# zhangkao/IIP_UAVSal_Saliency

Hardware: AMD Instinct MI355X
Metric: saliency frames/sec at 360x640 (higher is better)
Workload: dtype f32; 1 GPU; 360x640 batch=1 clip(s)/GPU seq=8, UAVSal.forward_clips, prec=f32, launch loop; requests_in_flight=1, clips_per_gpu=1, seq_len=8, height=360, width=640, precision=f32, persistent_state=False, parallelism=single GPU, fused_dw=10

## Files before the change

iip_uavsal_saliency_amd/_lib.py:

```python
from __future__ import annotations

import collections
import ctypes as C
import os

PKG = os.path.dirname(os.path.abspath(__file__))
LIB_PATH = os.environ.get("UAVSAL_HIP_LIB") or os.path.join(PKG, "libuavsal_hip.so")

PREC = {"f32": 0, "bf16x3": 1, "bf16": 2, "f16x3": 3}
ACT_NONE, ACT_RELU6, ACT_SIGMOID = 0, 1, 2
EPI_AFFINE, EPI_TWA, EPI_LSTM = 0, 1, 2
SK_TICKET_BASE = 4096

_ERR = {-1: "UAVSAL_EINVAL (null pointer / non-positive size)",
        -2: "UAVSAL_EALIGN (channel count / ld / pointer not 16-byte aligned)",
        -3: "UAVSAL_ESHAPE (shape not supported by the kernel)",
        -4: "UAVSAL_ESTATE (plan used in the wrong state)",
        -5: "UAVSAL_EDEVICE (a kernel reported a device-side error; the run's outputs are invalid)"}
ERR_STREAMK = 1
DW_KERNEL = {1: "dw3x3_kernel<1, 4, 4>", 2: "dw3x3_kernel<1, 2, 2>", 3: "dw3x3_kernel<2, 2, 2>", 4: "dw3x3_dilated_kernel",
             16: "dw3x3_map_lds_kernel<16, 256>", 32: "dw3x3_map_lds_kernel<32, 256>",
             528: "dw3x3_map_lds_kernel<16, 512>", 544: "dw3x3_map_lds_kernel<32, 512>",
             2048: "dw3x3_rowclass_kernel<256>"}

# ... 191 lines not shown
    _fields_ = [("g", _f), ("ldg", C.c_int32), ("carry", _f), ("z", _f), ("x", _f), ("ldx", C.c_int32),
                ("hprev", _f), ("ldh", C.c_int32), ("dz", _f), ("carry_out", _f), ("dx", _f),
                ("n_pix", C.c_int64), ("C", C.c_int32)]


class TwaWgradDesc(C.Structure):
    _fields_ = [("dz", _f), ("x", _f), ("ldx", C.c_int32), ("h", _f), ("ldh", C.c_int32), ("h0", _f), ("ldh0", C.c_int32),
                ("ws", _f), ("ws_bytes", C.c_int64), ("out", _f),
                ("T", C.c_int32), ("H", C.c_int32), ("W", C.c_int32), ("C", C.c_int32), ("accumulate", C.c_int32)]


class DecBwdDesc(C.Structure):
    _fields_ = [("gy", _f), ("gy_img_pitch", C.c_int64), ("gy_row_pitch", C.c_int64), ("gy_col_pitch", C.c_int64),
                ("y", _f), ("e", _f), ("d", _f), ("s1", _f), ("wd9", _f), ("s2", _f), ("w3", _f), ("s3", _f), ("ge", _f),
                ("n_img", C.c_int32), ("H", C.c_int32), ("W", C.c_int32), ("C", C.c_int32)]


TRAIN_DESC_TYPES = [TwaGateDesc, TwaWgradDesc, DecBwdDesc]

class PixGemmDesc(C.Structure):
    _fields_ = [("a", _f), ("lda", C.c_int32), ("b", _f), ("ldb", C.c_int32), ("row_scale", _f),
                ("w", _f), ("ldw", C.c_int32), ("rowdot", C.c_void_p), ("ws", _f), ("ws_bytes", C.c_int64),
                ("out", _f), ("ldo", C.c_int32), ("K", C.c_int64), ("M", C.c_int32), ("N", C.c_int32), ("accumulate", C.c_int32)]


class DecSumsDesc(C.Structure):
    _fields_ = [("gy", _f), ("gy_img_pitch", C.c_int64), ("gy_row_pitch", C.c_int64), ("gy_col_pitch", C.c_int64),
                ("y", _f), ("e", _f), ("d", _f), ("ga", _f), ("w3", _f), ("s3", _f),
                ("ws", C.c_void_p), ("ws_bytes", C.c_int64),
                ("n_img", C.c_int32), ("H", C.c_int32), ("W", C.c_int32), ("C", C.c_int32)]


class DecFinishDesc(C.Structure):
    _fields_ = [("ws", C.c_void_p), ("ws_bytes", C.c_int64), ("rowdot", C.c_void_p)] + [(n, _f) for n in (
        "wd", "w3", "s2", "s3", "r1", "mu1", "r2", "mu2", "r3", "mu3",
        "g_gamma1", "g_beta1", "g_wd", "g_gamma2", "g_beta2", "g_w3", "g_gamma3", "g_beta3")] + [
        ("C", C.c_int32), ("slabs", C.c_int32), ("accumulate", C.c_int32)]


DEC_NSUM = 12
TRAIN_DECODER_DESC_TYPES = [PixGemmDesc, DecSumsDesc, DecFinishDesc]

DESC_TYPES = [ConvDesc, DwDesc, StemDesc, BilinearDesc, TdiffDesc, TsumDesc, LayoutDesc, PostDesc, GuardDesc, CopyDesc,
              FusedIrDesc, WinoDesc, DwDotDesc, FillDesc, ScoreDesc, LetterboxDesc, OverlayDesc, GazeDesc, LossDesc, ConvRoute]

SYMBOLS = [
    ("uavsal_conv_gemm", C.c_int, [C.POINTER(ConvDesc), C.c_void_p]),
    ("uavsal_conv_route_of", C.c_int, [C.POINTER(ConvDesc), C.POINTER(ConvRoute)]),
    ("uavsal_conv_tile", C.c_int, [C.POINTER(ConvDesc)]),
    ("uavsal_conv_uses_split", C.c_int, [C.POINTER(ConvDesc)]),
    ("uavsal_conv_dwproj", C.c_int, [C.POINTER(ConvDesc)]),
    ("uavsal_streamk_workspace_bytes", C.c_longlong, []),
    ("uavsal_conv_streamk_grid", C.c_int, [C.POINTER(ConvDesc)]),
    ("uavsal_dw3x3", C.c_int, [C.POINTER(DwDesc), C.c_void_p]),
    ("uavsal_dw3x3_dot", C.c_int, [C.POINTER(DwDotDesc), C.c_void_p]),
    ("uavsal_dw_variant", C.c_int, [C.POINTER(DwDesc)]),
    ("uavsal_stem_conv", C.c_int, [C.POINTER(StemDesc), C.c_void_p]),
    ("uavsal_bilinear_ac", C.c_int, [C.POINTER(BilinearDesc), C.c_void_p]),
    ("uavsal_tdiff", C.c_int, [C.POINTER(TdiffDesc), C.c_void_p]),
    ("uavsal_tsum", C.c_int, [C.POINTER(TsumDesc), C.c_void_p]),
    ("uavsal_layout", C.c_int, [C.POINTER(LayoutDesc), C.c_void_p]),
    ("uavsal_postprocess", C.c_int, [C.POINTER(PostDesc), C.c_void_p]),
    ("uavsal_letterbox_u8", C.c_int, [C.POINTER(LetterboxDesc), C.c_void_p]),
    ("uavsal_overlay_workspace_bytes", C.c_int64, [C.POINTER(OverlayDesc)]),
    ("uavsal_overlay_u8", C.c_int, [C.POINTER(OverlayDesc), C.c_void_p]),
    ("uavsal_gaze_prepare", C.c_int, [C.POINTER(GazeDesc), C.c_void_p]),
    ("uavsal_loss_fu", C.c_int, [C.POINTER(LossDesc), C.c_void_p]),
    ("uavsal_loss_fu_grad", C.c_int, [C.POINTER(LossDesc), C.c_void_p]),
    ("uavsal_prior_accumulate", C.c_int, [C.POINTER(PriorAccDesc), C.c_void_p]),
    ("uavsal_prior_finish", C.c_int, [C.POINTER(PriorFinishDesc), C.c_void_p]),
    ("uavsal_prior_slab_frames", C.c_int, [C.c_int64, C.c_int32]),
    ("uavsal_prior_sizeof_desc", C.c_int, [C.c_int]),
    ("uavsal_twa_gate_bwd", C.c_int, [C.POINTER(TwaGateDesc), C.c_void_p]),
    ("uavsal_twa_wgrad_workspace_bytes", C.c_int64, [C.POINTER(TwaWgradDesc)]),
    ("uavsal_twa_wgrad_shares", C.c_int, [C.POINTER(TwaWgradDesc)]),
    ("uavsal_twa_wgrad", C.c_int, [C.POINTER(TwaWgradDesc), C.c_void_p]),
    ("uavsal_dec_bwd", C.c_int, [C.POINTER(DecBwdDesc), C.c_void_p]),
    ("uavsal_train_sizeof_desc", C.c_int, [C.c_int]),
    ("uavsal_pix_gemm_workspace_bytes", C.c_int64, [C.POINTER(PixGemmDesc)]),
    ("uavsal_pix_gemm_shares", C.c_int, [C.POINTER(PixGemmDesc)]),
    ("uavsal_pix_gemm", C.c_int, [C.POINTER(PixGemmDesc), C.c_void_p]),
    ("uavsal_dec_sums_workspace_bytes", C.c_int64, [C.POINTER(DecSumsDesc)]),
    ("uavsal_dec_sums_slabs", C.c_int, [C.POINTER(DecSumsDesc)]),
    ("uavsal_dec_sums_slab_rows", C.c_int, [C.POINTER(DecSumsDesc)]),
    ("uavsal_dec_sums", C.c_int, [C.POINTER(DecSumsDesc), C.c_void_p]),
    ("uavsal_dec_finish", C.c_int, [C.POINTER(DecFinishDesc), C.c_void_p]),
    ("uavsal_train_decoder_sizeof_desc", C.c_int, [C.c_int]),
    ("uavsal_guard", C.c_int, [C.POINTER(GuardDesc), C.c_void_p]),
    ("uavsal_copy_rows", C.c_int, [C.POINTER(CopyDesc), C.c_void_p]),
    ("uavsal_fill", C.c_int, [C.POINTER(FillDesc), C.c_void_p]),
    ("uavsal_plan_add_fill", C.c_int, [C.c_void_p, C.POINTER(FillDesc)]),
    ("uavsal_fused_ir", C.c_int, [C.POINTER(FusedIrDesc), C.c_void_p]),
    ("uavsal_fused_ir_supported", C.c_int, [C.POINTER(FusedIrDesc)]),
    ("uavsal_plan_add_fused_ir", C.c_int, [C.c_void_p, C.POINTER(FusedIrDesc)]),
    ("uavsal_wino_input", C.c_int, [C.POINTER(WinoDesc), C.c_void_p]),
    ("uavsal_wino_output", C.c_int, [C.POINTER(WinoDesc), C.c_void_p]),
    ("uavsal_plan_add_wino_input", C.c_int, [C.c_void_p, C.POINTER(WinoDesc)]),
    ("uavsal_plan_add_wino_output", C.c_int, [C.c_void_p, C.POINTER(WinoDesc)]),
    ("uavsal_plan_add_copy", C.c_int, [C.c_void_p, C.POINTER(CopyDesc)]),
    ("uavsal_plan_create", C.c_void_p, []),
    ("uavsal_plan_destroy", None, [C.c_void_p]),
    ("uavsal_plan_add_conv", C.c_int, [C.c_void_p, C.POINTER(ConvDesc)]),
    ("uavsal_plan_add_dw", C.c_int, [C.c_void_p, C.POINTER(DwDesc)]),
    ("uavsal_plan_add_dw_dot", C.c_int, [C.c_void_p, C.POINTER(DwDotDesc)]),
    ("uavsal_plan_add_stem", C.c_int, [C.c_void_p, C.POINTER(StemDesc)]),
    ("uavsal_plan_add_bilinear", C.c_int, [C.c_void_p, C.POINTER(BilinearDesc)]),
# ... 68 lines not shown
```

iip_uavsal_saliency_amd/build.py:

```python
from __future__ import annotations

import hashlib
import os
import subprocess
import sys
from concurrent.futures import ThreadPoolExecutor

PKG = os.path.dirname(os.path.abspath(__file__))
ROOT = os.path.dirname(PKG)
CSRC = os.path.join(PKG, "csrc")
INCLUDE = os.path.join(ROOT, "include")
LIB = os.path.join(PKG, "libuavsal_hip.so")
SOURCES = ["conv_gemm.hip", "conv_gemm_k32.hip", "dwproj.hip", "dw_conv.hip", "fused_ir.hip", "fused_mid.hip", "glue.hip", "letterbox.hip", "loss.hip", "overlay.hip", "post.hip", "plan.hip", "prior.hip", "score.hip", "train.hip", "train_decoder.hip", "winograd.hip"]
FLAGS = ["-O3", "--offload-arch=gfx950", "-std=c++17", "-fPIC", "-I" + INCLUDE, "-I" + CSRC]
FLAGS += os.environ.get("UAVSAL_EXTRA_HIPCC_FLAGS", "").split()


def _hipcc() -> str:
    for c in (os.environ.get("HIPCC"), "/opt/rocm/bin/hipcc", "hipcc"):
        if c and (os.path.isabs(c) and os.path.exists(c) or not os.path.isabs(c)):
            return c
    return "hipcc"


def _digest(paths, extra="") -> str:
    h = hashlib.sha256(extra.encode())
    for p in paths:
        h.update(os.path.basename(p).encode())
        with open(p, "rb") as f:
            h.update(f.read())
    return h.hexdigest()


def _stamp_ok(stamp: str, digest: str, target: str) -> bool:
    try:
        return os.path.exists(target) and open(stamp).read().strip() == digest
    except OSError:
        return False


def build(force: bool = False, verbose: bool = False) -> str:
    headers = sorted(os.path.join(CSRC, f) for f in os.listdir(CSRC) if f.endswith(".h"))
    headers += sorted(os.path.join(INCLUDE, f) for f in os.listdir(INCLUDE) if f.endswith(".h"))
    objs, jobs = [], []
    for src in SOURCES:
        s = os.path.join(CSRC, src)
        o = os.path.join(CSRC, src.replace(".hip", ".o"))
        objs.append(o)
        digest = _digest([s] + headers, " ".join(FLAGS))
        if force or not _stamp_ok(o + ".stamp", digest, o):
            jobs.append(([_hipcc()] + FLAGS + ["-c", s, "-o", o], o + ".stamp", digest))

    def run(job):
        cmd, stamp, digest = job
        if verbose:
            print(" ".join(cmd), flush=True)
        if stamp and os.path.exists(stamp):
            os.remove(stamp)
        r = subprocess.run(cmd, capture_output=True, text=True)
        if r.returncode != 0:
            raise RuntimeError("hipcc failed:\n%s\n%s" % (" ".join(cmd), r.stderr[-4000:]))
        if stamp:
            with open(stamp, "w") as f:
                f.write(digest)

    if jobs:
# ... 11 lines not shown
```

iip_uavsal_saliency_amd/csrc/conv_gemm.hip:

```cpp
#include <stdlib.h>
#include <type_traits>
#include "common.h"

#include "conv_gemm_common.h"
#include "conv_route.h"

namespace {

template <int PREC, int WAVES_M, int WAVES_N, int WM, int WN, int TAPS, bool FUSE = false>
__global__ __launch_bounds__(WAVES_M * WAVES_N * 64,
                             (WM * WN >= 4) ? ((PREC == UAVSAL_PREC_BF16X3 || PREC == UAVSAL_PREC_F16X3 || WAVES_M * WAVES_N == 8) ? 2 : 3) : 4)
void conv_gemm_kernel(const ConvK p) {
    constexpr int NT = WAVES_M * WAVES_N * 64;
    constexpr int NS = NT;
    static_assert(!FUSE || TAPS == 1, "the fused depthwise producer feeds a 1x1 projection");
    constexpr int BM = WAVES_M * WM * 32;
    constexpr int BN = WAVES_N * WN * 32;
    constexpr int KT = (PREC == UAVSAL_PREC_F32) ? 16 : 32;
    constexpr int NPAN = (PREC == UAVSAL_PREC_BF16X3 || PREC == UAVSAL_PREC_F16X3) ? 2 : 1;
    constexpr int NLD = (PREC == UAVSAL_PREC_F32) ? 1 : 2;
    constexpr int A_IT = (BM * 4) / NS;
    constexpr int B_IT = (BN * 4 + NS - 1) / NS;
    constexpr int APAN = BM * 64;
    constexpr int BPAN = BN * 64;
// ... 1087 lines not shown
    if (d->w_group_stride && !((tile == 8 || tile == 11) && k32_eligible(d, tile) && d->epi == UAVSAL_EPI_AFFINE && !d->a_split))
        status = UAVSAL_ESHAPE;
    else if (d->n_group < 0 || (d->n_group && !(k32_eligible(d, 11) && !d->a_split && !d->out_split)))
        status = UAVSAL_ESHAPE;
    const int ktiles = d->prec == UAVSAL_PREC_F32 ? (d->taps * d->Cin + 15) / 16 : (d->taps * d->Cin + 31) / 32;
    if (split_eligible(d, tile)) {
        r->family = UAVSAL_ROUTE_PRESPLIT;
        return status;
    }
    if (dwproj_eligible(d)) {
        r->family = UAVSAL_ROUTE_DWPROJ;
        r->dwproj = d->Cout > 128 ? 256 : (d->Cout > 64 ? 128 : (d->Cout > 32 ? 64 : 32));
        r->ksplit = dwproj_shares(d);
    } else if ((r->streamk = tile == 1 && sk1 >= 0 ? sk1 : streamk_plan(d, tile, ktiles)) > 0) {
        r->family = UAVSAL_ROUTE_STREAMK;
    } else if (tile >= 8 && tile <= 11) {
        r->family = UAVSAL_ROUTE_K32;
        r->ksplit = tile == 11 ? k32s_shares(d) : k32_shares(d, tile);
    } else if (d->prec == UAVSAL_PREC_F32 && !d->dw_w9c) {
        r->family = UAVSAL_ROUTE_F32_DMA;
    } else {
        r->family = UAVSAL_ROUTE_STAGED;
        r->ksplit = staged_shares(d, tile, ktiles);
    }
    if (r->ksplit > 1) r->reduce = r->family == UAVSAL_ROUTE_K32 && tile >= 10 ? UAVSAL_REDUCE_IN_LAUNCH : UAVSAL_REDUCE_LAUNCH;
    if (!status && r->family != UAVSAL_ROUTE_DWPROJ && !d->a) status = UAVSAL_EINVAL;
    return status;
}

extern "C" long long uavsal_streamk_workspace_bytes(void) {
    int dev = 0, n = 0;
    if (hipGetDevice(&dev) != hipSuccess ||
        hipDeviceGetAttribute(&n, hipDeviceAttributeMultiprocessorCount, dev) != hipSuccess || n <= 0) n = 256;
    const long long G = 2LL * n;
    return 65536 + G * 128 * 128 * 4;
}

extern "C" int uavsal_conv_route_of(const uavsal_conv_desc* d, uavsal_conv_route* r) {
    if (!d || !r || d->n_img <= 0 || d->H <= 0 || d->W <= 0 || d->Cout <= 0) return UAVSAL_EINVAL;
    (void)conv_route(d, r);
    return 0;
}

static uavsal_conv_route route_or_none(const uavsal_conv_desc* d, bool need_cin) {
    uavsal_conv_route r = {};
    if (d && (!need_cin || d->Cin > 0)) (void)uavsal_conv_route_of(d, &r);
    return r;
}
extern "C" int uavsal_conv_tile(const uavsal_conv_desc* d) { const int t = route_or_none(d, false).tile; return t ? t : UAVSAL_EINVAL; }
extern "C" int uavsal_conv_uses_split(const uavsal_conv_desc* d) { return route_or_none(d, true).family == UAVSAL_ROUTE_PRESPLIT; }
extern "C" int uavsal_conv_dwproj(const uavsal_conv_desc* d) { return route_or_none(d, true).dwproj; }
extern "C" int uavsal_conv_streamk_grid(const uavsal_conv_desc* d) { return route_or_none(d, true).streamk; }

extern "C" int uavsal_conv_gemm(const uavsal_conv_desc* d, uavsal_stream_t stream) {
    if (!d || !d->w || !d->out) return UAVSAL_EINVAL;
    if (!d->a && !(d->a_split && d->epi == UAVSAL_EPI_AFFINE)) return UAVSAL_EINVAL;
    if (d->n_img <= 0 || d->H <= 0 || d->W <= 0 || d->Cin <= 0 || d->Cout <= 0) return UAVSAL_EINVAL;
    if (d->taps != 1 && d->taps != 9) return UAVSAL_ESHAPE;
    if (d->prec < 0 || d->prec > 3) return UAVSAL_ESHAPE;
    if (d->Cin & 3) return UAVSAL_EALIGN;
    if (d->a && ((d->lda & 3) || d->lda < d->Cin || !uavsal_aligned16(d->a))) return UAVSAL_EALIGN;
    if (d->epi != UAVSAL_EPI_LSTM && d->ldc < d->Cout) return UAVSAL_ESHAPE;
    if (!uavsal_aligned16(d->w)) return UAVSAL_EALIGN;
    if (d->out_split && ((d->ldos & 63) || d->ldos < 2 * d->Cout || ((uintptr_t)d->out_split & 127)))
        return UAVSAL_EALIGN;
    if (d->out_split && d->prec != UAVSAL_PREC_F16X3) return UAVSAL_ESHAPE;
    uavsal_conv_route r;
    const int route_status = conv_route(d, &r);
    if (d->out_split) {
        const int t = r.tile;
        const bool twa_vec = d->epi == UAVSAL_EPI_TWA && (t == 3 || t == 4) && !(d->ldx & 3) && !(d->lda & 3) &&
                             uavsal_aligned16(d->aux);
        const bool vec = (d->epi == UAVSAL_EPI_AFFINE || twa_vec) && d->act != UAVSAL_ACT_SIGMOID && !(d->ldc & 3) &&
                         !(d->Cout & 3) && uavsal_aligned16(d->out) && (!d->res || (!(d->ldr & 3) && uavsal_aligned16(d->res)));
        if (!vec) return UAVSAL_ESHAPE;
    }
    if (d->taps == 9 && (d->Cin % 32)) return UAVSAL_ESHAPE;
    if ((d->scale == nullptr) != (d->bias == nullptr)) return UAVSAL_EINVAL;
    if (d->res && d->epi != UAVSAL_EPI_LSTM && d->ldr < d->Cout) return UAVSAL_ESHAPE;
    if (d->epi == UAVSAL_EPI_TWA) {
        if (!d->res || !d->aux || d->Cin != d->Cout || d->ldx < d->Cout) return UAVSAL_ESHAPE;
    } else if (d->epi == UAVSAL_EPI_LSTM) {
        if (!d->res || !d->aux || !d->out2 || (d->Cout & 3) || d->Cin * 4 != d->Cout) return UAVSAL_ESHAPE;
        if (d->ldc < d->Cin || d->ld2 < d->Cin || d->ldr < d->Cin || d->ldx < d->Cout) return UAVSAL_ESHAPE;
        if ((d->ldx & 3) || (d->ldc & 3) || (d->ldr & 3) || !uavsal_aligned16(d->aux) ||
            !uavsal_aligned16(d->out) || !uavsal_aligned16(d->res)) return UAVSAL_EALIGN;
    } else if (d->epi != UAVSAL_EPI_AFFINE) {
        return UAVSAL_ESHAPE;
    }
    const long long HW = (long long)d->H * d->W;
    const long long M = HW * d->n_img;
    if (M > 0x7fffffffLL) return UAVSAL_ESHAPE;
    if (d->dw_w9c) {
        if (d->taps != 1 || d->epi != UAVSAL_EPI_AFFINE || !d->dw_scale || !d->dw_bias) return UAVSAL_ESHAPE;
        if (d->dw_stride != 1 && d->dw_stride != 2) return UAVSAL_ESHAPE;
        if ((d->dw_Hin - 1) / d->dw_stride + 1 != d->H || (d->dw_Win - 1) / d->dw_stride + 1 != d->W) return UAVSAL_ESHAPE;
        if (d->a_img_stride < (long long)d->dw_Hin * d->dw_Win) return UAVSAL_ESHAPE;
        if (!uavsal_aligned16(d->dw_w9c) || !uavsal_aligned16(d->dw_scale) || !uavsal_aligned16(d->dw_bias)) return UAVSAL_EALIGN;
    } else if (d->a_img_stride < HW) {
        return UAVSAL_ESHAPE;
    }
    if (d->o_img_stride < HW) return UAVSAL_ESHAPE;

    ConvK k;
    k.a = d->a; k.w = (const char*)d->w; k.scale = d->scale; k.bias = d->bias;
    k.out = d->out; k.res = d->res; k.aux = d->aux; k.out2 = d->out2; k.ld2 = d->ld2;
    k.dw_w = d->dw_w9c; k.dw_s = d->dw_scale; k.dw_b = d->dw_bias;
    k.dw_stride = d->dw_stride; k.Hin = d->dw_Hin; k.Win = d->dw_Win;
    k.a_is = d->a_img_stride; k.o_is = d->o_img_stride;
    k.r_is = d->res ? d->r_img_stride : HW; k.x_is = d->aux ? d->x_img_stride : HW;
    k.lda = d->lda; k.ldc = d->ldc; k.ldr = d->ldr; k.ldx = d->ldx;
    k.M = (int)M; k.HW = (int)HW; k.H = d->H; k.W = d->W; k.Cin = d->Cin; k.Cout = d->Cout;
    const int KT = d->prec == UAVSAL_PREC_F32 ? 16 : 32;
    k.Kpad = (d->taps * d->Cin + KT - 1) / KT * KT;
    k.Npad = (d->Cout + 31) / 32 * 32;
    k.ktiles = k.Kpad / KT;
    if ((long long)k.Npad * k.Kpad * 4 > 0x7fffffffLL) return UAVSAL_ESHAPE;
    k.act = d->act; k.epi = d->epi;
    k.contig = ((k.a_is == HW || k.dw_w) && k.o_is == HW && k.r_is == HW && k.x_is == HW) ? 1 : 0;
    k.tiles_n = 0; k.nblk = 0;
    k.sk_part = nullptr; k.sk_flag = nullptr; k.err = nullptr; k.ksplit = r.ksplit; k.kpart = nullptr; k.kpart_bytes = 0;
    k.sk_spin = d->sk_spin_limit > 0 ? d->sk_spin_limit : (1 << 22);
    k.sk_drop = d->sk_debug_drop;
    k.w_gs = d->w_group_stride;
    k.ngrp = d->n_group; k.a_goff = d->a_group_off;
    k.a_sp = (const _Float16*)d->a_split; k.ldas = d->ldas;
    k.out_sp = (_Float16*)d->out_split; k.ldos = d->ldos;
    if (route_status) return route_status;
    hipStream_t s = (hipStream_t)stream;
    const bool t1 = d->taps == 1;
    if (r.family != UAVSAL_ROUTE_PRESPLIT && uavsal_route::kpart_room(d)) {
        k.kpart = (float*)((char*)d->sk_ws + 65536);
        k.kpart_bytes = d->sk_ws_bytes - 65536;
    }
    switch (r.family) {
        case UAVSAL_ROUTE_PRESPLIT: return launch_h16(k, d->taps, r.tile, s);
        case UAVSAL_ROUTE_DWPROJ: return uavsal_launch_dwproj(k, d->prec, r.dwproj, s);
        case UAVSAL_ROUTE_STREAMK:
            k.sk_flag = (int*)d->sk_ws;
            k.sk_part = (float*)((char*)d->sk_ws + 65536);
            k.err = d->err ? d->err : (int*)d->sk_ws + UAVSAL_SK_ERR_WORD;
            if (r.tile == 1) return t1 ? SkBig::launch<1>(k, r.streamk, s) : SkBig::launch<9>(k, r.streamk, s);
            if (r.tile == 3) return t1 ? SkThin::launch<1>(k, r.streamk, s) : SkThin::launch<9>(k, r.streamk, s);
            return t1 ? SkSmall::launch<1>(k, r.streamk, s) : SkSmall::launch<9>(k, r.streamk, s);
        case UAVSAL_ROUTE_K32:
            if (k.kpart) k.sk_flag = (int*)d->sk_ws + UAVSAL_SK_TICKET_BASE;
            return uavsal_launch_f32_k32(k, d->taps, r.tile, s);
        case UAVSAL_ROUTE_F32_DMA: return launch_f32(k, d->taps, r.tile, s);
        default: break;
    }
    switch (d->prec) {
        case UAVSAL_PREC_F32: return launch_prec<UAVSAL_PREC_F32>(k, d->taps, r.tile, s);
        case UAVSAL_PREC_BF16X3: return launch_prec<UAVSAL_PREC_BF16X3>(k, d->taps, r.tile, s);
        case UAVSAL_PREC_F16X3: return launch_prec<UAVSAL_PREC_F16X3>(k, d->taps, r.tile, s);
        default: return launch_prec<UAVSAL_PREC_BF16>(k, d->taps, r.tile, s);
    }
}
```

iip_uavsal_saliency_amd/csrc/conv_gemm_common.h:

```cpp
#pragma once
#include <stdlib.h>
#include <type_traits>
#include "common.h"

namespace uavsal_gemm {

struct ConvK {
    const float* a;
    const char* w;
    const float* scale;
    const float* bias;
    float* out;
    const float* res;
    const float* aux;
    float* out2;
    const float* dw_w; const float* dw_s; const float* dw_b;
    int dw_stride, Hin, Win;
    long long a_is, o_is, r_is, x_is;
    int lda, ldc, ldr, ldx, ld2;
    int M, HW, H, W, Cin, Cout, Kpad, Npad, ktiles, act, epi;
    int tiles_n, nblk, contig;
    float* sk_part;
    int* sk_flag;
    int* err;
    int sk_spin, sk_drop;
    int ksplit;
    float* kpart;
    long long kpart_bytes;
    const _Float16* a_sp;
    _Float16* out_sp;
    int ldas, ldos;
    long long w_gs;
    int ngrp, a_goff;
};

}

int uavsal_launch_f32_k32(const uavsal_gemm::ConvK& k, int taps, int tile, hipStream_t stream);
int uavsal_launch_dwproj(const uavsal_gemm::ConvK& k, int prec, int bn, hipStream_t stream);

namespace {
using uavsal_gemm::ConvK;

__device__ __forceinline__ long long row_off(int m, int HW, long long img_stride, int contig) {
    if (contig) return m;
    const int img = m / HW;
    return (long long)img * img_stride + (m - img * HW);
}

#define F16X3_A_SCALE 16.0f
#define F16X3_ACC_SCALE (1.0f / 1024.0f)

template <int PREC>
__device__ __forceinline__ unsigned pack2(float a, float b) {
    typedef float f2 __attribute__((ext_vector_type(2)));
    f2 v = {a, b};
    if (PREC == UAVSAL_PREC_F16X3) {
        typedef _Float16 h2 __attribute__((ext_vector_type(2)));
        h2 r = __builtin_convertvector(v, h2);
        return __builtin_bit_cast(unsigned, r);
    } else {
        typedef __bf16 bf2 __attribute__((ext_vector_type(2)));
        bf2 r = __builtin_convertvector(v, bf2);
        return __builtin_bit_cast(unsigned, r);
    }
}

template <int PREC>
__device__ __forceinline__ float hi_as_f32(float x) {
    if (PREC == UAVSAL_PREC_F16X3) { _Float16 h = (_Float16)x; return (float)h; }
    __bf16 h = (__bf16)x;
    return (float)h;
}

template <int PREC>
__device__ __forceinline__ f32x4 prescale(f32x4 x) {
    if (PREC == UAVSAL_PREC_F16X3) {
        x = x * F16X3_A_SCALE;
        x.x = fminf(fmaxf(x.x, -65504.f), 65504.f); x.y = fminf(fmaxf(x.y, -65504.f), 65504.f);
        x.z = fminf(fmaxf(x.z, -65504.f), 65504.f); x.w = fminf(fmaxf(x.w, -65504.f), 65504.f);
    }
    return x;
}

#ifndef UAVSAL_EPI_BARRIER
#define UAVSAL_EPI_BARRIER() __syncthreads()
#endif
#define UAVSAL_GEMM_EPILOGUE(ACC_SCALE, STG, SPLIT_OUT)                                                       \
    {                                                                                                \
         \
        const bool twa_ = (WM * WN == 1) && p.epi == UAVSAL_EPI_TWA;                                 \
        const bool lstm_ = (WM * WN == 1) && p.epi == UAVSAL_EPI_LSTM;                               \
// ... 207 lines not shown
```

iip_uavsal_saliency_amd/csrc/conv_route.h:

```cpp
#pragma once
#include "conv_gemm_common.h"

namespace uavsal_route {

inline long long rows(const uavsal_conv_desc* d) { return (long long)d->H * d->W * d->n_img; }
inline int npad(const uavsal_conv_desc* d) { return (d->Cout + 31) / 32 * 32; }
inline long long tiles(const uavsal_conv_desc* d, int bm, int bn) { return ((rows(d) + bm - 1) / bm) * ((d->Cout + bn - 1) / bn); }
inline long long kpart_room(const uavsal_conv_desc* d) {
    return d->sk_ws && uavsal_aligned16(d->sk_ws) && d->sk_ws_bytes > 65536 ? d->sk_ws_bytes - 65536 : 0;
}

inline int k32_share_count(long long tiles, int stages) {
    if (tiles <= 0 || tiles * 2 > 512) return 1;
    int ksp = (int)(512 / tiles);
    if (ksp > 4) ksp = 4;
    while (ksp > 1 && stages / ksp < 6) --ksp;
    return ksp;
}

inline bool k32_split_gates(const uavsal_conv_desc* d, long long ntiles) {
    if (!kpart_room(d) || (d->epi != UAVSAL_EPI_AFFINE && d->epi != UAVSAL_EPI_TWA) || d->act == UAVSAL_ACT_SIGMOID) return false;
    if (ntiles <= 0 || ntiles >= UAVSAL_SK_TICKET_MAX) return false;
    if ((d->Cout & 3) || (d->ldc & 3) || !uavsal_aligned16(d->out)) return false;
    if (d->res && ((d->ldr & 3) || !uavsal_aligned16(d->res))) return false;
// ... 5 lines not shown
    const long long ntiles = tiles(d, tile == 9 ? 256 : 128, 128);
    if (!k32_split_gates(d, ntiles) || 8LL * rows(d) * npad(d) * 4 > kpart_room(d)) return 1;
    return k32_share_count(ntiles, d->taps * d->Cin / 32);
}

inline int k32s_shares(const uavsal_conv_desc* d) {
    const long long ntiles = tiles(d, 64, 64);
    if (!k32_split_gates(d, ntiles)) return 1;
    int ksp = (int)(1024 / ntiles);
    if (ksp > 4) ksp = 4;
    while (ksp > 1 && d->taps * d->Cin / 32 / ksp < 4) --ksp;
    if (ksp < 1 || ntiles * ksp * 64 * 64 * 4 > kpart_room(d)) ksp = 1;
    return ksp;
}

inline bool k32_eligible(const uavsal_conv_desc* d, int tile) {
    if (tile < 8 || tile > 11) return false;
    if (d->w_group_stride && ((tile != 8 && tile != 11) || d->taps != 1 || (((long long)d->H * d->W) & 127))) return false;
    if (d->n_group && (tile != 11 || d->taps != 1 || d->w_group_stride || d->epi != UAVSAL_EPI_AFFINE || (d->n_group & 63) ||
                       d->Cout % d->n_group || d->a_group_off < d->Cin || (d->a_group_off & 3) ||
                       (long long)d->lda < (long long)(d->Cout / d->n_group - 1) * d->a_group_off + d->Cin)) return false;
    if (d->prec != UAVSAL_PREC_F32 || d->dw_w9c || d->epi == UAVSAL_EPI_LSTM) return false;
    if (tile == 11 && d->epi == UAVSAL_EPI_TWA && ((d->ldx & 3) || (d->lda & 3) || (d->ldc & 3) || (d->Cout & 3))) return false;
    if ((d->Cin % 32) || d->Cin > UAVSAL_DWPROJ_MAX_C) return false;
    if (tile == 10 && k32_shares(d, 10) <= 1 &&
        !(d->epi == UAVSAL_EPI_AFFINE && d->scale && d->bias && d->act != UAVSAL_ACT_SIGMOID && !(d->ldc & 3) && !(d->Cout & 3) &&
          uavsal_aligned16(d->out) && (!d->res || (!(d->ldr & 3) && uavsal_aligned16(d->res)))))
        return false;
    return d->taps == 1 || d->taps == 9;
}

inline int staged_shares(const uavsal_conv_desc* d, int tile, int ktiles) {
    if ((tile != 3 && tile != 4) || !kpart_room(d) || d->dw_w9c || (d->prec != UAVSAL_PREC_F16X3 && d->prec != UAVSAL_PREC_BF16X3) ||
        !(d->epi == UAVSAL_EPI_AFFINE || (d->epi == UAVSAL_EPI_TWA && d->taps == 9)))
        return 1;
    const long long ntiles = tile == 3 ? tiles(d, 128, 32) : tiles(d, 64, 64);
    int ksp = (int)(1024 / (ntiles > 0 ? ntiles : 1));
    ksp = ksp >= 4 ? 4 : (ksp >= 2 ? 2 : 1);
    while (ksp > 1 && (ktiles % (d->taps * ksp) || ktiles / ksp < (d->taps == 1 ? 12 : 18))) ksp >>= 1;
    const bool ok = (long long)ksp * rows(d) * npad(d) * 4 <= kpart_room(d) && !(d->Cout & 3) && !(d->ldc & 3) &&
                    (d->epi != UAVSAL_EPI_TWA || (!(d->ldx & 3) && !(d->lda & 3) && !(d->ldr & 3)));
    return ok ? ksp : 1;
}

inline int dwproj_shares(const uavsal_conv_desc* d) {
    if (d->Cout > 32 || !kpart_room(d)) return 1;
    const long long ntiles = (long long)d->n_img * ((d->H + 7) / 8) * ((d->W + 15) / 16);
    int ksp = (int)(512 / (ntiles > 0 ? ntiles : 1));
    if (ksp > 4) ksp = 4;
    while (ksp > 1 && (d->Cin / 16) / ksp < 12) --ksp;
    return ksp > 1 && (long long)ksp * rows(d) * npad(d) * 4 <= kpart_room(d) ? ksp : 1;
}

}
```

iip_uavsal_saliency_amd/ops.py:

```python
from __future__ import annotations

import ctypes as C
from typing import Optional

import torch

from . import _lib as L
from . import packing as P


def _stream(t):
    return C.c_void_p(torch.cuda.current_stream(t.device).cuda_stream)


def _nhwc_view(t: torch.Tensor):
    if t.dim() != 4 or t.dtype != torch.float32 or not t.is_cuda:
        raise RuntimeError("expected a float32 cuda NHWC tensor [n,h,w,c]")
    n, h, w, c = t.shape
    ld = t.stride(2) if w > 1 else (t.stride(1) if h > 1 else (t.stride(0) if n > 1 else c))
    ok = (c == 1 or t.stride(3) == 1) and (w == 1 or t.stride(2) == ld) \
        and (h == 1 or t.stride(1) == w * ld) and (n == 1 or t.stride(0) == h * w * ld)
    if not ok:
        raise RuntimeError("tensor is not an NHWC buffer (or channel slice of one)")
    return t.data_ptr(), ld, n, h, w, c
# ... 35 lines not shown
    lib = L.load()
    ap, lda, n, hin, win, cin = _nhwc_view(x)
    stride = dw[3] if dw is not None else 1
    h, w = (hin - 1) // stride + 1, (win - 1) // stride + 1
    cout, taps = weight.shape[0], weight.shape[2] * weight.shape[3]
    if n_group:
        cin = weight.shape[1]
    if out is None:
        out = torch.empty((n, h, w, cout), dtype=torch.float32, device=x.device)
    op, ldc, *_ = _nhwc_view(out)
    keep = []
    d = L.ConvDesc()
    d.n_group, d.a_group_off = n_group, (cin if n_group else 0)
    d.a, d.lda, d.a_img_stride = ap, lda, hin * win
    if split_in:
        if not x.is_contiguous():
            raise RuntimeError("split_in needs a dense NHWC tensor")
        xs = split_shadow(x)
        keep.append(xs)
        d.a_split, d.ldas = xs.data_ptr(), 2 * cin
    shadow = None
    if split_out:
        shadow = _empty_shadow(n, h, w, cout, x.device)
        d.out_split, d.ldos = shadow.data_ptr(), 2 * cout
    if dw is not None:
        w9 = P.pack_dw_weight(dw[0]).to(x.device)
        ds, db = dw[1].float().contiguous().to(x.device), dw[2].float().contiguous().to(x.device)
        keep += [w9, ds, db]
        d.dw_w9c, d.dw_scale, d.dw_bias = w9.data_ptr(), ds.data_ptr(), db.data_ptr()
        d.dw_stride, d.dw_Hin, d.dw_Win = stride, hin, win
    if scale is not None:
        npad = P.roundup(cout, 32)
        s = P.pad_vec(scale, npad, 1.0).to(x.device)
        b = P.pad_vec(bias, npad, 0.0).to(x.device)
        keep += [s, b]
        d.scale, d.bias = s.data_ptr(), b.data_ptr()
    d.out, d.ldc, d.o_img_stride = op, ldc, h * w
    if res is not None:
        rp, ldr, *_ = _nhwc_view(res)
        d.res, d.ldr, d.r_img_stride = rp, ldr, h * w
    d.n_img, d.H, d.W, d.Cin, d.Cout, d.taps = n, h, w, cin, cout, taps
    d.prec, d.act, d.epi, d.tile = L.PREC[prec], act, L.EPI_AFFINE, tile
    if stream_k or dw is not None:
        ws = torch.zeros(int(lib.uavsal_streamk_workspace_bytes()), dtype=torch.uint8, device=x.device)
        keep.append(ws)
        d.sk_ws, d.sk_ws_bytes = ws.data_ptr(), ws.numel()
        d.sk_spin_limit, d.sk_debug_drop = sk_spin_limit, sk_debug_drop
        if _stale_streamk_flags:
            ws[:4 * L.SK_TICKET_BASE].view(torch.int32).fill_(1)
    d.w = 1 << 20
    rt = L.conv_route(lib, d)
    if route is not None:
        route.update(rt._asdict())
    uses_split = rt.family == L.ROUTE_PRESPLIT
    if split_in and not uses_split:
        raise RuntimeError("this shape / tile does not take the pre-split path")
    wp = P.pack_conv_weight(weight, P.conv_weight_layout(prec, uses_split, rt.dwproj != 0, rt.tile, weight.shape[-1])).to(x.device)
    keep.append(wp)
    d.w = wp.data_ptr()
    L.check(lib.uavsal_conv_gemm(C.byref(d), _stream(x)), "uavsal_conv_gemm")
    torch.cuda.current_stream(x.device).synchronize()
    if stream_k and not _stale_streamk_flags:
        _streamk_outcome(ws, "uavsal_conv_gemm")
    return (out, shadow) if split_out else out


def conv3x3_winograd(x, weight, scale=None, bias=None, act=L.ACT_NONE, res=None, twa=None, r=2, size=None):
    lib = L.load()
    segs = None
    if isinstance(x, (list, tuple)):
        segs = [_nhwc_view(t) for t in x]
        n, (h, w), cin = segs[0][2], size, sum(sg[5] for sg in segs)
        ip, ldi, x = None, 0, x[0]
    else:
        ip, ldi, n, h, w, cin = _nhwc_view(x)
    cout = weight.shape[0]
    tiles = n * ((h + r - 1) // r) * ((w + r - 1) // r)
    pp = (r + 2) * (r + 2)
    mp = P.roundup(tiles, 128)
    dev = x.device
    v = torch.zeros((pp, mp, cin), dtype=torch.float32, device=dev)
    m = torch.empty((pp, mp, cout), dtype=torch.float32, device=dev)
    out = torch.empty((n, h, w, cout), dtype=torch.float32, device=dev)
    wp = P.pack_wino_weight(weight, r).to(dev)
    st = _stream(x)
    wi = L.WinoDesc()
    wi.inp, wi.ldi, wi.out, wi.ldo = ip, ldi, v.data_ptr(), cin
    wi.n_img, wi.H, wi.W, wi.C, wi.Mp, wi.R = n, h, w, cin, mp, r
    if segs is not None:
        wi.n_seg = len(segs)
        for i, (sp_, sld_, sn_, sh_, sw_, sc_) in enumerate(segs):
            wi.seg_in[i], wi.seg_ld[i], wi.seg_c[i], wi.seg_H[i], wi.seg_W[i] = sp_, sld_, sc_, sh_, sw_
    L.check(lib.uavsal_wino_input(C.byref(wi), st), "uavsal_wino_input")
    d = L.ConvDesc()
    d.a, d.lda, d.a_img_stride = v.data_ptr(), cin, mp
    d.w = wp.data_ptr()
    d.w_group_stride = P.roundup(cout, 32) * P.roundup(cin, 32)
    d.out, d.ldc, d.o_img_stride = m.data_ptr(), cout, mp
    d.n_img, d.H, d.W, d.Cin, d.Cout, d.taps = pp, mp, 1, cin, cout, 1
    d.prec, d.act, d.epi, d.tile = L.PREC["f32"], L.ACT_NONE, L.EPI_AFFINE, 0
    L.check(lib.uavsal_conv_gemm(C.byref(d), st), "uavsal_conv_gemm(winograd planes)")
    wo = L.WinoDesc()
    wo.inp, wo.ldi, wo.out, wo.ldo = m.data_ptr(), cout, out.data_ptr(), cout
    wo.n_img, wo.H, wo.W, wo.C, wo.Mp, wo.R = n, h, w, cout, mp, r
    keep = [v, m, wp]
    if scale is not None:
# ... 393 lines not shown
```

include/uavsal_hip.h:

```cpp
#ifndef UAVSAL_HIP_H
#define UAVSAL_HIP_H

#include <stdint.h>

#ifdef __cplusplus
extern "C" {
#endif

#define UAVSAL_ABI_VERSION 20

#define UAVSAL_EINVAL   (-1)
#define UAVSAL_EALIGN   (-2)
#define UAVSAL_ESHAPE   (-3)
#define UAVSAL_ESTATE   (-4)
#define UAVSAL_EDEVICE  (-5)

#define UAVSAL_ERR_STREAMK  1

#define UAVSAL_PREC_F32     0
#define UAVSAL_PREC_BF16X3  1
#define UAVSAL_PREC_BF16    2
#define UAVSAL_PREC_F16X3   3

#define UAVSAL_ACT_NONE     0
#define UAVSAL_ACT_RELU6    1
#define UAVSAL_ACT_SIGMOID  2

#define UAVSAL_EPI_AFFINE   0
#define UAVSAL_EPI_TWA      1
#define UAVSAL_EPI_LSTM     2

typedef void* uavsal_stream_t;

typedef struct uavsal_conv_desc {
    const float* a;      int32_t lda;  int64_t a_img_stride;
    const void*  w;
    const float* scale;  const float* bias;
    float*       out;    int32_t ldc;  int64_t o_img_stride;
    const float* res;    int32_t ldr;  int64_t r_img_stride;
    const float* aux;    int32_t ldx;  int64_t x_img_stride;
    int32_t n_img, H, W;
    int32_t Cin, Cout, taps;
    int32_t prec, act, epi;
    int32_t tile;
    float*       out2;   int32_t ld2;
    const float* dw_w9c; const float* dw_scale; const float* dw_bias;
    int32_t dw_stride, dw_Hin, dw_Win;
    void* sk_ws; int64_t sk_ws_bytes;
    const void* a_split;  int32_t ldas;
    void* out_split;      int32_t ldos;
    int32_t* err;
    int32_t sk_spin_limit;
    int32_t sk_debug_drop;
    int64_t w_group_stride;
    int32_t n_group, a_group_off;
} uavsal_conv_desc;

int uavsal_conv_gemm(const uavsal_conv_desc* d, uavsal_stream_t stream);
long long uavsal_streamk_workspace_bytes(void);

enum { UAVSAL_ROUTE_PRESPLIT = 1, UAVSAL_ROUTE_DWPROJ, UAVSAL_ROUTE_STREAMK, UAVSAL_ROUTE_K32, UAVSAL_ROUTE_F32_DMA,
       UAVSAL_ROUTE_STAGED };
enum { UAVSAL_REDUCE_NONE = 0, UAVSAL_REDUCE_LAUNCH, UAVSAL_REDUCE_IN_LAUNCH };
typedef struct uavsal_conv_route {
    int32_t family;
    int32_t tile;
    int32_t dwproj;
    int32_t streamk;
    int32_t ksplit;
    int32_t reduce;
} uavsal_conv_route;
int uavsal_conv_route_of(const uavsal_conv_desc* d, uavsal_conv_route* r);
int uavsal_conv_tile(const uavsal_conv_desc* d);
int uavsal_conv_uses_split(const uavsal_conv_desc* d);
int uavsal_conv_dwproj(const uavsal_conv_desc* d);
int uavsal_conv_streamk_grid(const uavsal_conv_desc* d);

typedef struct uavsal_dw_desc {
    const float* in;   int32_t ldi;
    const float* w9c;  const float* scale;  const float* bias;
    float*       out;  int32_t ldo;
    int32_t n_img, H, W, C, stride, dilation, act;
    void* out_split;  int32_t ldos;
    int32_t dil_group_c;  int32_t dil_groups[4];
} uavsal_dw_desc;

int uavsal_dw3x3(const uavsal_dw_desc* d, uavsal_stream_t stream);
int uavsal_dw_variant(const uavsal_dw_desc* d);

typedef struct uavsal_dw_dot_desc {
    const float* in;   int32_t ldi;
    const float* w9c;  const float* scale;  const float* bias;
    const float* w2;   const float* scale2; const float* bias2;
    float*       out;  int32_t ldo;
    int32_t n_img, H, W, C, act;
} uavsal_dw_dot_desc;

int uavsal_dw3x3_dot(const uavsal_dw_dot_desc* d, uavsal_stream_t stream);

typedef struct uavsal_fused_ir_desc {
    const float* in;   int32_t ldi;
    const float* w1;   const float* scale1;  const float* bias1;
    const float* wd;   const float* scale_d; const float* bias_d;
    const float* w2;   const float* scale2;  const float* bias2;
    const float* res;  int32_t ldr;
    float*       out;  int32_t ldo;
    int32_t n_img, H, W, Cin, hidden, Cout, stride;
    int32_t tile;
} uavsal_fused_ir_desc;

int uavsal_fused_ir(const uavsal_fused_ir_desc* d, uavsal_stream_t stream);
int uavsal_fused_ir_supported(const uavsal_fused_ir_desc* d);

typedef struct uavsal_stem_desc {
    const float*   in;
    const uint8_t* in_u8;
    const float* w;  const float* scale;  const float* bias;
    float* out;  int32_t ldo;
    int32_t n_img, H, W;
    float mean[3], stdv[3];
} uavsal_stem_desc;

int uavsal_stem_conv(const uavsal_stem_desc* d, uavsal_stream_t stream);

typedef struct uavsal_bilinear_desc {
    const float* in;  int32_t ldi;  int32_t Hi, Wi;
    float* out;       int32_t ldo;  int32_t Ho, Wo;
    int32_t n_out, C, src_mod, src_div;
    void* out_split;  int32_t ldos;
// ... 285 lines not shown
```

Baseline: 1933 frames/s.

## Add persistent weight-resident streaming kernel for large f32 1x1 convolutions

Adds a new persistent kernel for f32 1x1 convs with small output widths (32/64/256/384 padded columns) on the F32_DMA/K32 routes. It keeps the whole packed weight matrix resident in LDS, gives each wave a contiguous range of 32-row slabs, streams activations through a per-wave ring with direct global-to-LDS loads, and fuses the affine, ReLU6 and residual epilogue. The aim is to remove repeated weight loads and per-tile launch and sync overhead on memory-bound projections. In exchange it needs one 512-thread block per CU holding 160 KB of LDS, uses hand-tuned vmcnt waits, and only applies above row-count thresholds.

After: 1932 frames/s. Within noise of the previous version (-0.0%).

```diff
diff --git a/iip_uavsal_saliency_amd/_lib.py b/iip_uavsal_saliency_amd/_lib.py
--- a/iip_uavsal_saliency_amd/_lib.py
+++ b/iip_uavsal_saliency_amd/_lib.py
@@ -267,6 +267,7 @@
     ("uavsal_conv_dwproj", C.c_int, [C.POINTER(ConvDesc)]),
     ("uavsal_streamk_workspace_bytes", C.c_longlong, []),
     ("uavsal_conv_streamk_grid", C.c_int, [C.POINTER(ConvDesc)]),
+    ("uavsal_conv_streams", C.c_int, [C.POINTER(ConvDesc)]),
     ("uavsal_dw3x3", C.c_int, [C.POINTER(DwDesc), C.c_void_p]),
     ("uavsal_dw3x3_dot", C.c_int, [C.POINTER(DwDotDesc), C.c_void_p]),
     ("uavsal_dw_variant", C.c_int, [C.POINTER(DwDesc)]),
diff --git a/iip_uavsal_saliency_amd/build.py b/iip_uavsal_saliency_amd/build.py
--- a/iip_uavsal_saliency_amd/build.py
+++ b/iip_uavsal_saliency_amd/build.py
@@ -11,7 +11,7 @@
 CSRC = os.path.join(PKG, "csrc")
 INCLUDE = os.path.join(ROOT, "include")
 LIB = os.path.join(PKG, "libuavsal_hip.so")
-SOURCES = ["conv_gemm.hip", "conv_gemm_k32.hip", "dwproj.hip", "dw_conv.hip", "fused_ir.hip", "fused_mid.hip", "glue.hip", "letterbox.hip", "loss.hip", "overlay.hip", "post.hip", "plan.hip", "prior.hip", "score.hip", "train.hip", "train_decoder.hip", "winograd.hip"]
+SOURCES = ["conv_gemm.hip", "conv_gemm_k32.hip", "conv_stream.hip", "dwproj.hip", "dw_conv.hip", "fused_ir.hip", "fused_mid.hip", "glue.hip", "letterbox.hip", "loss.hip", "overlay.hip", "post.hip", "plan.hip", "prior.hip", "score.hip", "train.hip", "train_decoder.hip", "winograd.hip"]
 FLAGS = ["-O3", "--offload-arch=gfx950", "-std=c++17", "-fPIC", "-I" + INCLUDE, "-I" + CSRC]
 FLAGS += os.environ.get("UAVSAL_EXTRA_HIPCC_FLAGS", "").split()
 
diff --git a/iip_uavsal_saliency_amd/csrc/conv_gemm.hip b/iip_uavsal_saliency_amd/csrc/conv_gemm.hip
--- a/iip_uavsal_saliency_amd/csrc/conv_gemm.hip
+++ b/iip_uavsal_saliency_amd/csrc/conv_gemm.hip
@@ -1163,6 +1163,16 @@
 extern "C" int uavsal_conv_dwproj(const uavsal_conv_desc* d) { return route_or_none(d, true).dwproj; }
 extern "C" int uavsal_conv_streamk_grid(const uavsal_conv_desc* d) { return route_or_none(d, true).streamk; }
 
+static bool conv_streams(const uavsal_conv_desc* d, const uavsal_conv_route& r) {
+    return uavsal_route::stream_eligible(d) && (r.family == UAVSAL_ROUTE_F32_DMA || r.family == UAVSAL_ROUTE_K32) &&
+           r.ksplit <= 1 && r.streamk <= 0;
+}
+extern "C" int uavsal_conv_streams(const uavsal_conv_desc* d) {
+    uavsal_conv_route r = {};
+    if (!d || d->Cin <= 0 || uavsal_conv_route_of(d, &r) != 0) return 0;
+    return conv_streams(d, r) ? 1 : 0;
+}
+
 extern "C" int uavsal_conv_gemm(const uavsal_conv_desc* d, uavsal_stream_t stream) {
     if (!d || !d->w || !d->out) return UAVSAL_EINVAL;
     if (!d->a && !(d->a_split && d->epi == UAVSAL_EPI_AFFINE)) return UAVSAL_EINVAL;
@@ -1244,6 +1254,7 @@
         k.kpart = (float*)((char*)d->sk_ws + 65536);
         k.kpart_bytes = d->sk_ws_bytes - 65536;
     }
+    if (conv_streams(d, r)) return uavsal_launch_conv_stream(k, s);
     switch (r.family) {
         case UAVSAL_ROUTE_PRESPLIT: return launch_h16(k, d->taps, r.tile, s);
         case UAVSAL_ROUTE_DWPROJ: return uavsal_launch_dwproj(k, d->prec, r.dwproj, s);
diff --git a/iip_uavsal_saliency_amd/csrc/conv_gemm_common.h b/iip_uavsal_saliency_amd/csrc/conv_gemm_common.h
--- a/iip_uavsal_saliency_amd/csrc/conv_gemm_common.h
+++ b/iip_uavsal_saliency_amd/csrc/conv_gemm_common.h
@@ -38,6 +38,8 @@
 
 int uavsal_launch_f32_k32(const uavsal_gemm::ConvK& k, int taps, int tile, hipStream_t stream);
 int uavsal_launch_dwproj(const uavsal_gemm::ConvK& k, int prec, int bn, hipStream_t stream);
+
+int uavsal_launch_conv_stream(const uavsal_gemm::ConvK& k, hipStream_t stream);
 
 namespace {
 using uavsal_gemm::ConvK;
diff --git a/iip_uavsal_saliency_amd/csrc/conv_route.h b/iip_uavsal_saliency_amd/csrc/conv_route.h
--- a/iip_uavsal_saliency_amd/csrc/conv_route.h
+++ b/iip_uavsal_saliency_amd/csrc/conv_route.h
@@ -81,4 +81,41 @@
     return ksp > 1 && (long long)ksp * rows(d) * npad(d) * 4 <= kpart_room(d) ? ksp : 1;
 }
 
+struct stream_shape { int cols, wn, cs; };
+inline int stream_instance(int npad) { return npad == 32 ? 0 : (npad == 64 ? 1 : (npad == 256 ? 2 : (npad == 384 ? 3 : -1))); }
+inline stream_shape stream_shape_of(int inst) {
+    const stream_shape s[4] = {{32, 1, 1}, {64, 2, 1}, {256, 4, 2}, {384, 6, 2}};
+    return s[inst];
 }
+constexpr int STREAM_LDS_BYTES = 160 * 1024;
+constexpr int STREAM_WAVES = 8;
+inline int stream_ring_units(int npad, bool res) { return npad <= 64 && !res ? 4 : 2; }
+inline long long stream_weight_bytes(const uavsal_conv_desc* d) { return (long long)((d->Cin + 31) / 32) * npad(d) * 128; }
+constexpr int stream_res_pieces(int wn) { return wn % 2 == 0 ? 4 : 2; }
+inline long long stream_weight_room(int npad_, bool res) {
+    const int pieces = stream_res_pieces(stream_shape_of(stream_instance(npad_)).wn);
+    return STREAM_LDS_BYTES - (long long)STREAM_WAVES * (stream_ring_units(npad_, res) * 4096 + (res ? pieces * 2048 : 0));
+}
+inline long long stream_min_rows(int npad_, bool res) {
+#ifdef UAVSAL_STREAM_MIN_ROWS
+    return UAVSAL_STREAM_MIN_ROWS;
+#else
+    return npad_ <= 64 ? 230400 : (res ? 28800 : 57600);
+#endif
+}
+inline bool stream_eligible(const uavsal_conv_desc* d) {
+    if (d->prec != UAVSAL_PREC_F32 || d->taps != 1 || d->epi != UAVSAL_EPI_AFFINE) return false;
+    if (d->tile != 0 && d->tile != 11) return false;
+    if (d->act != UAVSAL_ACT_NONE && d->act != UAVSAL_ACT_RELU6) return false;
+    if (d->n_group || d->w_group_stride || d->dw_w9c || d->a_split || d->out_split) return false;
+    const long long HW = (long long)d->H * d->W;
+    if (d->a_img_stride != HW || d->o_img_stride != HW || (d->res && d->r_img_stride != HW)) return false;
+    if (d->Cin <= 0 || (d->Cin % 16) || (d->Cout & 3)) return false;
+    if ((d->lda & 3) || (d->ldc & 3) || !d->a || !uavsal_aligned16(d->a) || !uavsal_aligned16(d->out)) return false;
+    if (d->res && ((d->ldr & 3) || !uavsal_aligned16(d->res))) return false;
+    if ((d->scale == nullptr) != (d->bias == nullptr)) return false;
+    if (stream_instance(npad(d)) < 0 || stream_weight_bytes(d) > stream_weight_room(npad(d), d->res != nullptr)) return false;
+    return rows(d) >= stream_min_rows(npad(d), d->res != nullptr) && rows(d) <= 0x7fffffffLL - 512;
+}
+
+}
diff --git a/iip_uavsal_saliency_amd/csrc/conv_stream.hip b/iip_uavsal_saliency_amd/csrc/conv_stream.hip
--- /dev/null
+++ b/iip_uavsal_saliency_amd/csrc/conv_stream.hip
@@ -0,0 +1,210 @@
+#include "conv_gemm_common.h"
+#include "conv_route.h"
+
+namespace {
+
+template <int N>
+__device__ __forceinline__ void vm_wait() {
+    asm volatile("s_waitcnt vmcnt(%0)" ::"n"(N < 63 ? N : 63) : "memory");
+}
+
+template <int WN, int CS, int NU, bool RES>
+__global__ __launch_bounds__(512, 1) void conv_stream_kernel(const ConvK p) {
+    constexpr int NW = uavsal_route::STREAM_WAVES;
+    constexpr int UNIT = 32 * 128;
+    constexpr int LPU = 4;
+    constexpr int AH = NU - 1;
+    constexpr int PIECES = 2 * WN;
+    constexpr int E = PIECES * (RES ? 4 : 2);
+    constexpr int P = uavsal_route::stream_res_pieces(WN);
+    static_assert(NU == 2 || NU == 4, "the waits below know these two rings");
+    static_assert(CS == 1 || CS == 2, "one wave or a pair per slab");
+
+    extern __shared__ __attribute__((aligned(16))) char smem[];
+    typedef const __attribute__((address_space(1))) void* gptr_t;
+    typedef __attribute__((address_space(3))) void* lptr_t;
+
+    const int tid = threadIdx.x;
+    const int wave_u = __builtin_amdgcn_readfirstlane(tid >> 6);
+    const int lane = tid & 63;
+    const int lr = lane & 31, lh = lane >> 5;
+    const int KU = (p.Kpad + 31) >> 5;
+    const int nuu_last = (p.Kpad & 16) ? 2 : 4;
+    char* ring = smem + wave_u * (NU * UNIT);
+    char* rbuf = smem + NW * NU * UNIT + wave_u * (P * 2048);
+    char* wlds = smem + NW * NU * UNIT + (RES ? NW * P * 2048 : 0);
+
+    size_t zero_page = (size_t)g_zero16;
+    asm volatile("" : "+s"(zero_page));
+
+    const int n0 = (CS == 2 ? (wave_u & 1) : 0) * (WN * 32);
+    float sc[WN], bi[WN];
+#pragma unroll
+    for (int j = 0; j < WN; ++j) {
+        const int col = n0 + j * 32 + lr;
+        const bool okn = p.scale != nullptr && col < p.Cout;
+        sc[j] = okn ? p.scale[col] : 1.f;
+        bi[j] = okn ? p.bias[col] : 0.f;
+    }
+    const float lo = p.act == UAVSAL_ACT_RELU6 ? 0.f : -3.0e38f;
+    const float hi = p.act == UAVSAL_ACT_RELU6 ? 6.f : 3.0e38f;
+
+    const int nworkers = (int)gridDim.x * (NW / CS);
+    const int worker = xcd_virtual_block(blockIdx.x, gridDim.x) * (NW / CS) + wave_u / CS;
+    int s = (int)(((long long)p.nblk * worker) / nworkers);
+    const int s_end = (int)(((long long)p.nblk * (worker + 1)) / nworkers);
+    const bool has_work = s < s_end;
+    const int total = has_work ? (s_end - s) * KU : 0;
+    const int l8 = lane >> 3;
+
+    int i_s = s, i_ku = 0, i_slot = 0;
+    auto issue_unit = [&]() {
+        char* dst = ring + i_slot * UNIT;
+#pragma unroll
+        for (int it = 0; it < LPU; ++it) {
+            const int kf = i_ku * 32 + (((lane & 7) ^ (((it & 1) << 2) | (l8 >> 1))) << 2);
+            const bool kin = kf < p.Cin && i_s < s_end;
+            const int m = i_s * 32 + it * 8 + l8;
+            const size_t src = (kin && m < p.M) ? (size_t)(p.a + (long long)m * p.lda + kf) : zero_page;
+            __builtin_amdgcn_global_load_lds((gptr_t)src, (lptr_t)(dst + it * 1024), 16, 0, 0);
+        }
+        if (++i_ku == KU) { i_ku = 0; ++i_s; }
+        i_slot = (i_slot + 1 == NU) ? 0 : i_slot + 1;
+    };
+    int q_s = s, q_j = 0;
+    auto issue_piece = [&](int hb, int sl) {
+        const int c = n0 + q_j * 32 + (lane & 7) * 4;
+        const int cc = c < p.Cout ? c : 0;
+#pragma unroll
+        for (int it = 0; it < 2; ++it) {
+            int m = q_s * 32 + hb * 16 + it * 8 + l8;
+            m = m < p.M ? m : p.M - 1;
+            const float* src = p.res + (long long)m * p.ldr + cc;
+            __builtin_amdgcn_global_load_lds((gptr_t)src, (lptr_t)(rbuf + sl * 2048 + it * 1024), 16, 0, 0);
+        }
+        if (hb == 1 && ++q_j == WN) { q_j = 0; ++q_s; }
+    };
+    if (has_work) {
+        if constexpr (RES) {
+#pragma unroll
+            for (int q = 0; q < P; ++q) issue_piece(q & 1, q);
+        }
+#pragma unroll
+        for (int t = 0; t < AH; ++t) issue_unit();
+    }
+
+    const int r8 = tid >> 3;
+    const int lc4 = ((tid & 7) ^ ((r8 >> 1) & 7)) * 4;
+    for (int ku = 0; ku < KU; ++ku) {
+        const bool kin = ku * 32 + lc4 < p.Kpad;
+        for (int it = 0; it * 64 + wave_u * 8 < p.Npad; ++it) {
+            const int n = it * 64 + r8;
+            const size_t src = kin ? (size_t)(reinterpret_cast<const float*>(p.w) + (size_t)n * p.Kpad + ku * 32 + lc4) : zero_page;
+            __builtin_amdgcn_global_load_lds((gptr_t)src, (lptr_t)(wlds + ((size_t)ku * p.Npad + it * 64 + wave_u * 8) * 128), 16, 0, 0);
+        }
+    }
+#pragma unroll
+    for (int j = 0; j < WN; ++j) asm volatile("" : "+v"(sc[j]), "+v"(bi[j]));
+    asm volatile("s_waitcnt vmcnt(0)" ::: "memory");
+    asm volatile("s_waitcnt lgkmcnt(0)\n\ts_barrier" ::: "memory");
+    if (!has_work) return;
+
+
+    const int sw = (lr >> 1) & 7;
+    const int a_row = lr * 128;
+    const char* b_row = wlds + (size_t)(n0 + lr) * 128;
+    f32x16 acc[WN];
+    int ku = 0, slot = 0;
+    for (int g = 0; g < total; ++g) {
+        if constexpr (NU == 2) {
+            const bool epi_before = g > 0 && ku == 0;
+            if (epi_before) vm_wait<E>(); else vm_wait<0>();
+        } else {
+            if (KU == 1 && g >= 3) vm_wait<LPU * 2 + 3 * E>();
+            else if (KU == 1 && g == 2) vm_wait<LPU * 2 + 2 * E>();
+            else if (KU == 1 && g == 1) vm_wait<LPU * 2 + E>();
+            else vm_wait<LPU * 2>();
+        }
+        issue_unit();
+        const char* au = ring + slot * UNIT;
+        const char* wu = b_row + (size_t)ku * p.Npad * 128;
+        if (ku == 0) {
+#pragma unroll
+            for (int j = 0; j < WN; ++j)
+#pragma unroll
+                for (int r = 0; r < 16; ++r) acc[j][r] = 0.f;
+        }
+        const int nuu = ku == KU - 1 ? nuu_last : 4;
+#pragma unroll
+        for (int uu = 0; uu < 4; ++uu) {
+            if (uu < 2 || nuu == 4) {
+                const int so = ((2 * uu + lh) ^ sw) * 16;
+                const f32x4 av = *reinterpret_cast<const f32x4*>(au + a_row + so);
+                f32x4 bv[WN];
+#pragma unroll
+                for (int j = 0; j < WN; ++j) bv[j] = *reinterpret_cast<const f32x4*>(wu + j * 32 * 128 + so);
+#pragma unroll
+                for (int j = 0; j < WN; ++j) {
+                    acc[j] = __builtin_amdgcn_mfma_f32_32x32x2f32(av.x, bv[j].x, acc[j], 0, 0, 0);
+                    acc[j] = __builtin_amdgcn_mfma_f32_32x32x2f32(av.y, bv[j].y, acc[j], 0, 0, 0);
+                    acc[j] = __builtin_amdgcn_mfma_f32_32x32x2f32(av.z, bv[j].z, acc[j], 0, 0, 0);
+                    acc[j] = __builtin_amdgcn_mfma_f32_32x32x2f32(av.w, bv[j].w, acc[j], 0, 0, 0);
+                }
+            }
+        }
+        if (++ku == KU) {
+            ku = 0;
+            float* stg = reinterpret_cast<float*>(ring + slot * UNIT);
+#pragma unroll
+            for (int j = 0; j < WN; ++j) {
+#pragma unroll
+                for (int hb = 0; hb < 2; ++hb) {
+                    float* sh = stg + hb * 512;
+                    constexpr int PM = P - 1;
+                    const int sl = (j * 2 + hb) & PM;
+#pragma unroll
+                    for (int gg = 0; gg < 8; ++gg) {
+                        const int r16 = (gg & 3) + 8 * (gg >> 2) + 4 * lh;
+                        sh[r16 * 32 + lr] = __builtin_amdgcn_fmed3f(fmaf(acc[j][hb * 8 + gg], sc[j], bi[j]), lo, hi);
+                    }
+                    if constexpr (RES) {
+                        if (s * 32 + 32 > p.M) vm_wait<0>(); else vm_wait<4 * (P - 1)>();
+                    }
+                    const int gn = n0 + j * 32 + (lane & 7) * 4;
+#pragma unroll
+                    for (int it = 0; it < 2; ++it) {
+                        const int r16 = it * 8 + l8;
+                        f32x4 v = *reinterpret_cast<const f32x4*>(sh + r16 * 32 + (lane & 7) * 4);
+                        if constexpr (RES) v += *reinterpret_cast<const f32x4*>(rbuf + sl * 2048 + r16 * 128 + (lane & 7) * 16);
+                        const int gm = s * 32 + hb * 16 + r16;
+                        if (gm < p.M && gn < p.Cout) *reinterpret_cast<f32x4*>(p.out + (long long)gm * p.ldc + gn) = v;
+                    }
+                    if constexpr (RES) issue_piece(hb, sl);
+                }
+            }
+            ++s;
+        }
+        slot = (slot + 1 == NU) ? 0 : slot + 1;
+    }
+}
+
+template <int WN, int CS>
+int launch_stream(const ConvK& k, hipStream_t stream) {
+    constexpr int SMEM = uavsal_route::STREAM_LDS_BYTES;
+    if (k.res) return launch_resident<conv_stream_kernel<WN, CS, 2, true>, SMEM, 512, true>(k, stream);
+    return launch_resident<conv_stream_kernel<WN, CS, (WN * CS <= 2 ? 4 : 2), false>, SMEM, 512, true>(k, stream);
+}
+
+}
+
+int uavsal_launch_conv_stream(const ConvK& k0, hipStream_t stream) {
+    ConvK k = k0;
+    k.nblk = (k.M + 31) / 32;
+    switch (uavsal_route::stream_instance(k.Npad)) {
+        case 0: return launch_stream<1, 1>(k, stream);
+        case 1: return launch_stream<2, 1>(k, stream);
+        case 2: return launch_stream<4, 2>(k, stream);
+        case 3: return launch_stream<6, 2>(k, stream);
+        default: return UAVSAL_ESHAPE;
+    }
+}
diff --git a/iip_uavsal_saliency_amd/ops.py b/iip_uavsal_saliency_amd/ops.py
--- a/iip_uavsal_saliency_amd/ops.py
+++ b/iip_uavsal_saliency_amd/ops.py
@@ -111,6 +111,7 @@
     rt = L.conv_route(lib, d)
     if route is not None:
         route.update(rt._asdict())
+        route["streams"] = bool(lib.uavsal_conv_streams(C.byref(d)))
     uses_split = rt.family == L.ROUTE_PRESPLIT
     if split_in and not uses_split:
         raise RuntimeError("this shape / tile does not take the pre-split path")
diff --git a/include/uavsal_hip.h b/include/uavsal_hip.h
--- a/include/uavsal_hip.h
+++ b/include/uavsal_hip.h
@@ -75,6 +75,7 @@
 int uavsal_conv_uses_split(const uavsal_conv_desc* d);
 int uavsal_conv_dwproj(const uavsal_conv_desc* d);
 int uavsal_conv_streamk_grid(const uavsal_conv_desc* d);
+int uavsal_conv_streams(const uavsal_conv_desc* d);
 
 typedef struct uavsal_dw_desc {
     const float* in;   int32_t ldi;
```
